# jianzhnie/ScaleRL

Measured on AMD Instinct MI355X. Metric: env_steps_per_sec, higher is better.
Workload: dtype bf16; 1 GPU; model=IMPALA AtariNet (3conv+FC512+2xLSTM519), algo=impala-vtrace, rollout_length=80, global_batch=256, seq_len=80, envs_per_actor=256, actors_per_rank=24, inference=gpu, parallelism=dp1

## Files before the change

### scalerl_amd/models/atari.py

```python

from __future__ import annotations

from typing import Dict, Tuple

import torch
import torch.nn as nn
import torch.nn.functional as F

from ..ops import MaskedLSTM, frame_cast


class AtariNet(nn.Module):
    def __init__(self, observation_shape=(4, 84, 84), num_actions: int = 6,
                 use_lstm: bool = True, native_conv: bool = None):
        super().__init__()
        self.observation_shape = tuple(observation_shape)
        self.num_actions = num_actions
        self.use_lstm = use_lstm
        if native_conv is None:
            import os
            native_conv = bool(os.environ.get("SCALERL_NATIVE_CONV"))
        self.native_conv = native_conv and tuple(observation_shape) == (4, 84, 84)

        c = observation_shape[0]
        self.conv1 = nn.Conv2d(c, 32, kernel_size=8, stride=4)
        self.conv2 = nn.Conv2d(32, 64, kernel_size=4, stride=2)
        self.conv3 = nn.Conv2d(64, 64, kernel_size=3, stride=1)
        conv_out = 64 * 7 * 7
        self.fc = nn.Linear(conv_out, 512)

        core_output_size = 512 + num_actions + 1
        if use_lstm:
            self.core = MaskedLSTM(core_output_size, core_output_size,
                                   num_layers=2)
        self.policy = nn.Linear(core_output_size, num_actions)
        self.baseline = nn.Linear(core_output_size, 1)

    def initial_state(self, batch_size: int, device=None):
        if not self.use_lstm:
            return tuple()
        return self.core.initial_state(batch_size, device=device)

    def encode(self, x: torch.Tensor) -> torch.Tensor:
        if self.native_conv and x.is_cuda:
            from ..ops.conv import native_conv
            h = native_conv(1, x, self.conv1.weight, self.conv1.bias)
            h = native_conv(2, h, self.conv2.weight, self.conv2.bias)
            h = native_conv(3, h, self.conv3.weight, self.conv3.bias)
            return F.relu(self.fc(torch.flatten(h, 1)))
        if (x.is_cuda and x.dtype == torch.uint8 and
                frame_cast.bf16_autocast_active()):
            x = frame_cast.frame_to_bf16(x)
        else:
            x = x.float() / 255.0
        x = F.relu(self.conv1(x))
        x = F.relu(self.conv2(x))
        x = F.relu(self.conv3(x))
        x = torch.flatten(x, 1)
        return F.relu(self.fc(x))

    def forward(self, inputs: Dict[str, torch.Tensor],
                core_state: Tuple = (), greedy: bool = False):
        obs = inputs["obs"]
        T, B = obs.shape[:2]
        feat = self.encode(obs.flatten(0, 1))

        one_hot_action = F.one_hot(
            inputs["last_action"].view(T * B), self.num_actions).float()
        clipped_reward = torch.clamp(inputs["reward"].view(T * B, 1), -1, 1)
        core_input = torch.cat(
            [feat.float(), clipped_reward, one_hot_action], dim=-1)

        if self.use_lstm:
            notdone = (~inputs["done"].view(T, B)).float()
            core_output, core_state = self.core(
                core_input.view(T, B, -1), notdone, core_state)
            core_output = core_output.flatten(0, 1)
        else:
            core_output = core_input

        if core_output.is_cuda:
            with torch.autocast(device_type="cuda", enabled=False):
                policy_logits = self.policy(core_output.float())
                baseline = self.baseline(core_output.float())
        else:
            policy_logits = self.policy(core_output.float())
            baseline = self.baseline(core_output.float())
        if greedy or not self.training:
            action = torch.argmax(policy_logits, dim=-1)
        else:
            action = torch.multinomial(
                F.softmax(policy_logits, dim=-1), num_samples=1).squeeze(-1)
        return ({"policy_logits": policy_logits.view(T, B, self.num_actions),
                 "baseline": baseline.view(T, B),
                 "action": action.view(T, B)}, core_state)


class AtariQNet(nn.Module):

    def __init__(self, observation_shape=(4, 84, 84), num_actions: int = 6,
                 dueling: bool = True, noisy: bool = False):
        super().__init__()
        from .noisy import NoisyLinear
        c = observation_shape[0]
        self.num_actions = num_actions
        self.dueling = dueling
        self.noisy = noisy
        lin = NoisyLinear if noisy else nn.Linear
        self.conv1 = nn.Conv2d(c, 32, kernel_size=8, stride=4)
        self.conv2 = nn.Conv2d(32, 64, kernel_size=4, stride=2)
        self.conv3 = nn.Conv2d(64, 64, kernel_size=3, stride=1)
        self.fc = nn.Linear(64 * 7 * 7, 512)
        if dueling:
            self.value_head = lin(512, 1)
            self.adv_head = lin(512, num_actions)
        else:
            self.head = lin(512, num_actions)

    def reset_noise(self):
        from .noisy import reset_noise
        reset_noise(self)

    def forward(self, x: torch.Tensor) -> torch.Tensor:
        x = x.float() / 255.0
        x = F.relu(self.conv1(x))
        x = F.relu(self.conv2(x))
        x = F.relu(self.conv3(x))
        h = F.relu(self.fc(torch.flatten(x, 1)))
        if self.dueling:
            v = self.value_head(h)
            a = self.adv_head(h)
            return v + a - a.mean(dim=-1, keepdim=True)
        return self.head(h)


class CategoricalAtariQNet(nn.Module):

    def __init__(self, observation_shape=(4, 84, 84), num_actions: int = 6,
                 num_atoms: int = 51, v_min: float = -10.0,
                 v_max: float = 10.0, noisy: bool = False):
        super().__init__()
        from .noisy import NoisyLinear
        c = observation_shape[0]
        self.action_dim = self.num_actions = num_actions
        self.num_atoms = num_atoms
        self.noisy = noisy
        lin = NoisyLinear if noisy else nn.Linear
        self.conv1 = nn.Conv2d(c, 32, kernel_size=8, stride=4)
        self.conv2 = nn.Conv2d(32, 64, kernel_size=4, stride=2)
        self.conv3 = nn.Conv2d(64, 64, kernel_size=3, stride=1)
        self.fc = nn.Linear(64 * 7 * 7, 512)
        self.head = lin(512, num_actions * num_atoms)
        self.register_buffer("support", torch.linspace(v_min, v_max, num_atoms))
        self.v_min, self.v_max = v_min, v_max
        self.delta_z = (v_max - v_min) / (num_atoms - 1)

    def reset_noise(self):
        from .noisy import reset_noise
        reset_noise(self)

    def dist(self, x: torch.Tensor) -> torch.Tensor:
        x = x.float() / 255.0
        x = F.relu(self.conv1(x))
        x = F.relu(self.conv2(x))
        x = F.relu(self.conv3(x))
        h = F.relu(self.fc(torch.flatten(x, 1)))
        logits = self.head(h).view(-1, self.num_actions, self.num_atoms)
        return F.log_softmax(logits, dim=-1)

    def forward(self, x: torch.Tensor) -> torch.Tensor:
        return (self.dist(x).exp() * self.support).sum(-1)
```

### scalerl_amd/ops/__init__.py

```python

from ._backend import available as kernels_available
from ._backend import build as build_kernels
from .frame_cast import frame_to_bf16
from .lstm import MaskedLSTM
from .optim import FusedAdam, FusedRMSprop, clip_grad_norm_, fused_polyak_
from .per import SumTree
from .scans import discounted_returns, gae, nstep_fold
from .td import fused_td_loss, per_is_weights, td_loss_reference
from .ppo import ppo_fused_loss, ppo_loss_reference
from .vtrace import (VTraceReturns, action_log_probs, impala_loss,
                     impala_loss_reference, vtrace_from_log_rhos,
                     vtrace_reference)

__all__ = [
    "kernels_available", "build_kernels", "MaskedLSTM", "FusedAdam",
    "FusedRMSprop", "clip_grad_norm_", "fused_polyak_", "SumTree",
    "discounted_returns", "gae", "nstep_fold", "fused_td_loss",
    "per_is_weights", "td_loss_reference", "VTraceReturns",
    "action_log_probs", "impala_loss", "impala_loss_reference",
    "vtrace_from_log_rhos", "vtrace_reference", "ppo_fused_loss",
    "ppo_loss_reference", "frame_to_bf16",
]
```

### scalerl_amd/ops/csrc/frame_cast.hip

```cpp

#include "common.h"

#include <stdint.h>

__device__ __forceinline__ uint32_t frame_bf16_bits(uint32_t byte) {
  const float f = (float)byte * (1.0f / 255.0f);
  uint32_t u = __float_as_uint(f);
  u += 0x7fffu + ((u >> 16) & 1u);
  return u >> 16;
}

__device__ __forceinline__ uint32_t frame_bf16_pair(uint32_t word, int k) {
  const uint32_t lo = frame_bf16_bits((word >> (16 * k)) & 0xffu);
  const uint32_t hi = frame_bf16_bits((word >> (16 * k + 8)) & 0xffu);
  return lo | (hi << 16);
}

extern "C" __global__ void frame_cast_u8_bf16_kernel(
    const uint8_t* __restrict__ in,
    uint16_t* __restrict__ out,
    long n_vec,
    long n) {
  const long tid = (long)blockIdx.x * blockDim.x + threadIdx.x;
  const long stride = (long)gridDim.x * blockDim.x;
  const uint4* in4 = reinterpret_cast<const uint4*>(in);
  uint4* out4 = reinterpret_cast<uint4*>(out);
  for (long v = tid; v < n_vec; v += stride) {
    const uint4 p = in4[v];
    uint4 a, b;
    a.x = frame_bf16_pair(p.x, 0);
    a.y = frame_bf16_pair(p.x, 1);
    a.z = frame_bf16_pair(p.y, 0);
    a.w = frame_bf16_pair(p.y, 1);
    b.x = frame_bf16_pair(p.z, 0);
    b.y = frame_bf16_pair(p.z, 1);
    b.z = frame_bf16_pair(p.w, 0);
    b.w = frame_bf16_pair(p.w, 1);
    out4[2 * v] = a;
    out4[2 * v + 1] = b;
  }
  for (long i = n_vec * 16 + tid; i < n; i += stride)
    out[i] = (uint16_t)frame_bf16_bits(in[i]);
}

extern "C" int frame_cast_u8_bf16(const void* in, void* out, long n,
                                  hipStream_t stream) {
  if (n <= 0) return 0;
  const bool aligned =
      (((uintptr_t)in | (uintptr_t)out) & (uintptr_t)15) == 0;
  const long n_vec = aligned ? n / 16 : 0;
  const int block = 256;
  const long work = n_vec > 0 ? n_vec : n;
  hipLaunchKernelGGL(frame_cast_u8_bf16_kernel, dim3(grid_1d(work, block)),
                     dim3(block), 0, stream, (const uint8_t*)in,
                     (uint16_t*)out, n_vec, n);
  CHECK_LAUNCH();
  return 0;
}
```

Baseline: 419,100 env-steps/s.

## Fuse uint8 cast and three conv layers into one persistent MFMA encoder kernel

Adds a persistent HIP kernel that converts uint8 frames to bf16 in LDS and runs conv1, conv2 and conv3 with bias and ReLU using MFMA, keeping intermediate activations in shared memory. It also prefetches the next frame while computing. It is enabled by default on the inference (no-grad) path for actor forward passes, replacing the separate cast kernel and three conv launches with their global-memory round trips. Training stays on the old path unless an env flag is set, in which case a custom backward uses the saved activations. Weights are cast to bf16 on every call, which adds small per-call overhead.

New measurement: 494,600 env-steps/s (median of 6 runs). +18.0%, better.

```diff
diff --git a/scalerl_amd/models/atari.py b/scalerl_amd/models/atari.py
--- a/scalerl_amd/models/atari.py
+++ b/scalerl_amd/models/atari.py
@@ -1,6 +1,7 @@
 
 from __future__ import annotations
 
+import os
 from typing import Dict, Tuple
 
 import torch
@@ -8,17 +9,25 @@
 import torch.nn.functional as F
 
 from ..ops import MaskedLSTM, frame_cast
+from ..ops.encoder import fused_encoder
+
+FUSED_ENCODER = os.environ.get("SCALERL_FUSED_ENCODER", "1") != "0"
+FUSED_ENCODER_TRAIN = os.environ.get("SCALERL_FUSED_ENCODER_TRAIN", "0") == "1"
 
 
 class AtariNet(nn.Module):
     def __init__(self, observation_shape=(4, 84, 84), num_actions: int = 6,
-                 use_lstm: bool = True, native_conv: bool = None):
+                 use_lstm: bool = True, native_conv: bool = None,
+                 fused_encoder: bool = None):
         super().__init__()
         self.observation_shape = tuple(observation_shape)
         self.num_actions = num_actions
         self.use_lstm = use_lstm
+        if fused_encoder is None:
+            fused_encoder = native_conv is not False
+        self.fused_encoder = (bool(fused_encoder) and
+                              tuple(observation_shape) == (4, 84, 84))
         if native_conv is None:
-            import os
             native_conv = bool(os.environ.get("SCALERL_NATIVE_CONV"))
         self.native_conv = native_conv and tuple(observation_shape) == (4, 84, 84)
 
@@ -48,8 +57,16 @@
             h = native_conv(2, h, self.conv2.weight, self.conv2.bias)
             h = native_conv(3, h, self.conv3.weight, self.conv3.bias)
             return F.relu(self.fc(torch.flatten(h, 1)))
-        if (x.is_cuda and x.dtype == torch.uint8 and
-                frame_cast.bf16_autocast_active()):
+        bf16_frames = (x.is_cuda and x.dtype == torch.uint8 and
+                       frame_cast.bf16_autocast_active())
+        if (bf16_frames and self.fused_encoder and FUSED_ENCODER and
+                (FUSED_ENCODER_TRAIN or not torch.is_grad_enabled()) and
+                x.is_contiguous() and x.data_ptr() % 16 == 0):
+            h = fused_encoder(x, self.conv1.weight, self.conv1.bias,
+                              self.conv2.weight, self.conv2.bias,
+                              self.conv3.weight, self.conv3.bias)
+            return F.relu(self.fc(torch.flatten(h, 1)))
+        if bf16_frames:
             x = frame_cast.frame_to_bf16(x)
         else:
             x = x.float() / 255.0
diff --git a/scalerl_amd/ops/__init__.py b/scalerl_amd/ops/__init__.py
--- a/scalerl_amd/ops/__init__.py
+++ b/scalerl_amd/ops/__init__.py
@@ -1,6 +1,7 @@
 
 from ._backend import available as kernels_available
 from ._backend import build as build_kernels
+from .encoder import fused_encoder
 from .frame_cast import frame_to_bf16
 from .lstm import MaskedLSTM
 from .optim import FusedAdam, FusedRMSprop, clip_grad_norm_, fused_polyak_
@@ -19,5 +20,5 @@
     "per_is_weights", "td_loss_reference", "VTraceReturns",
     "action_log_probs", "impala_loss", "impala_loss_reference",
     "vtrace_from_log_rhos", "vtrace_reference", "ppo_fused_loss",
-    "ppo_loss_reference", "frame_to_bf16",
+    "ppo_loss_reference", "frame_to_bf16", "fused_encoder",
 ]
diff --git a/scalerl_amd/ops/csrc/encoder_fwd.hip b/scalerl_amd/ops/csrc/encoder_fwd.hip
--- /dev/null
+++ b/scalerl_amd/ops/csrc/encoder_fwd.hip
@@ -0,0 +1,302 @@
+
+#include "common.h"
+#include "frame_cast.h"
+
+typedef __bf16 bf16_t;
+typedef float f32x4 __attribute__((ext_vector_type(4)));
+typedef bf16_t bf16x8 __attribute__((ext_vector_type(8)));
+typedef bf16_t bf16x4 __attribute__((ext_vector_type(4)));
+typedef uint32_t u32x4 __attribute__((ext_vector_type(4)));
+
+namespace {
+
+constexpr int ENC_IMG_BYTES = 4 * 84 * 84;
+constexpr int ENC_CH_EL = 48 * 84;
+constexpr int ENC_IMG_EL = 4 * ENC_CH_EL;
+constexpr int ENC_ACT1_EL = 32 * 400;
+constexpr int ENC_P3 = 72;
+constexpr int ENC_ACT2_EL = 81 * ENC_P3;
+constexpr int ENC_OUT3_EL = 64 * 49;
+static_assert(ENC_ACT2_EL <= ENC_IMG_EL, "act2 aliases the image range");
+static_assert((ENC_IMG_EL + ENC_ACT1_EL + ENC_OUT3_EL) * 2 <= 65536,
+              "static LDS cap");
+
+template <int H>
+struct Half {
+  static constexpr int R0 = H ? 40 : 0;
+  static constexpr int NROWS = H ? 44 : 48;
+  static constexpr int VEC = NROWS * 84 / 16;
+  static constexpr int TILE0 = H ? 13 : 0;
+  static constexpr int NTILES = H ? 12 : 13;
+  static_assert(NROWS * 84 % 16 == 0 && R0 * 84 % 16 == 0, "16-byte chunks");
+  static_assert(VEC <= 256, "one load per thread and channel");
+};
+
+template <int H>
+__device__ __forceinline__ void load_half(const uint8_t* __restrict__ ximg,
+                                          uint4 (&pre)[4], int tid) {
+  if (tid < Half<H>::VEC) {
+    #pragma unroll
+    for (int c = 0; c < 4; ++c)
+      pre[c] = reinterpret_cast<const uint4*>(
+          ximg + c * (84 * 84) + Half<H>::R0 * 84)[tid];
+  }
+}
+
+template <int H>
+__device__ __forceinline__ void store_half(const uint4 (&pre)[4],
+                                           bf16_t* img, int tid) {
+  if (tid < Half<H>::VEC) {
+    #pragma unroll
+    for (int c = 0; c < 4; ++c) {
+      uint4 a, b;
+      frame_bf16_x16(pre[c], a, b);
+      uint4* dst = reinterpret_cast<uint4*>(img + c * ENC_CH_EL);
+      dst[2 * tid] = a;
+      dst[2 * tid + 1] = b;
+    }
+  }
+}
+
+__device__ __forceinline__ bf16x4 relu_bias_pack(const f32x4 acc, float bias) {
+  bf16x4 o;
+  #pragma unroll
+  for (int r = 0; r < 4; ++r) o[r] = (bf16_t)fmaxf(acc[r] + bias, 0.f);
+  return o;
+}
+
+template <int H>
+__device__ __forceinline__ void conv1_half(const bf16_t* img, bf16_t* act1,
+                                           const bf16x8 (&B1)[8], float bias,
+                                           int wave, int g, int lr) {
+  const int nt = wave >> 1;
+  for (int t = wave & 1; t < Half<H>::NTILES; t += 4) {
+    const bool two = t + 2 < Half<H>::NTILES;
+    const int tile[2] = {Half<H>::TILE0 + t,
+                         Half<H>::TILE0 + (two ? t + 2 : t)};
+    int base[2];
+    #pragma unroll
+    for (int i = 0; i < 2; ++i) {
+      const int px = tile[i] * 16 + lr;
+      const int oy = px / 20, ox = px - oy * 20;
+      base[i] = (oy * 4 - Half<H>::R0 + g) * 84 + ox * 4;
+    }
+    f32x4 acc[2] = {{0.f, 0.f, 0.f, 0.f}, {0.f, 0.f, 0.f, 0.f}};
+    #pragma unroll
+    for (int kt = 0; kt < 8; ++kt) {
+      const int off = (kt >> 1) * ENC_CH_EL + (kt & 1) * 4 * 84;
+      #pragma unroll
+      for (int i = 0; i < 2; ++i) {
+        const bf16x4* p = reinterpret_cast<const bf16x4*>(img + base[i] + off);
+        const bf16x8 a =
+            __builtin_shufflevector(p[0], p[1], 0, 1, 2, 3, 4, 5, 6, 7);
+        acc[i] = __builtin_amdgcn_mfma_f32_16x16x32_bf16(a, B1[kt], acc[i],
+                                                         0, 0, 0);
+      }
+    }
+    bf16_t* row = act1 + (nt * 16 + lr) * 400 + g * 4;
+    *reinterpret_cast<bf16x4*>(row + tile[0] * 16) =
+        relu_bias_pack(acc[0], bias);
+    if (two)
+      *reinterpret_cast<bf16x4*>(row + tile[1] * 16) =
+          relu_bias_pack(acc[1], bias);
+  }
+}
+
+template <bool SAVE>
+__global__ __launch_bounds__(256) __attribute__((amdgpu_waves_per_eu(2)))
+void atari_encoder_fwd_kernel(
+    const uint8_t* __restrict__ x,
+    const bf16_t* __restrict__ w1,
+    const float* __restrict__ b1,
+    const bf16_t* __restrict__ w2,
+    const float* __restrict__ b2,
+    const bf16_t* __restrict__ w3,
+    const float* __restrict__ b3,
+    bf16_t* __restrict__ out1,
+    bf16_t* __restrict__ out2,
+    bf16_t* __restrict__ out3,
+    long batch) {
+  __shared__ __attribute__((aligned(16)))
+  bf16_t lds[ENC_IMG_EL + ENC_ACT1_EL + ENC_OUT3_EL];
+  bf16_t* const img = lds;
+  bf16_t* const act2 = lds;
+  bf16_t* const act1 = lds + ENC_IMG_EL;
+  bf16_t* const o3 = lds + ENC_IMG_EL + ENC_ACT1_EL;
+
+  const int tid = threadIdx.x;
+  const int wave = tid >> 6;
+  const int lane = tid & (WAVE - 1);
+  const int g = lane >> 4, lr = lane & 15;
+
+  const int ch1 = (wave >> 1) * 16 + lr;
+  const int ch = wave * 16 + lr;
+  bf16x8 B1[8], B2[16], B3[18];
+  #pragma unroll
+  for (int kt = 0; kt < 8; ++kt)
+    B1[kt] = *reinterpret_cast<const bf16x8*>(w1 + ch1 * 256 + kt * 32 + g * 8);
+  #pragma unroll
+  for (int kt = 0; kt < 16; ++kt)
+    B2[kt] = *reinterpret_cast<const bf16x8*>(w2 + ch * 512 + kt * 32 + g * 8);
+  #pragma unroll
+  for (int kt = 0; kt < 18; ++kt) {
+    #pragma unroll
+    for (int j = 0; j < 8; ++j)
+      B3[kt][j] = w3[ch * 576 + ((kt & 1) * 32 + g * 8 + j) * 9 + (kt >> 1)];
+  }
+  const float bias1 = b1[ch1], bias2 = b2[ch], bias3 = b3[ch];
+
+  int base2[6], base3[4];
+  #pragma unroll
+  for (int mt = 0; mt < 6; ++mt) {
+    const int px = min(mt * 16 + lr, 80);
+    const int oy = px / 9, ox = px - oy * 9;
+    base2[mt] = (g >> 1) * 400 + (oy * 2 + (g & 1) * 2) * 20 + ox * 2;
+  }
+  #pragma unroll
+  for (int mt = 0; mt < 4; ++mt) {
+    const int px = min(mt * 16 + lr, 48);
+    const int oy = px / 7, ox = px - oy * 7;
+    base3[mt] = (oy * 9 + ox) * ENC_P3 + g * 8;
+  }
+
+  long n = blockIdx.x;
+  uint4 pre[4];
+  if (n < batch) load_half<0>(x + n * ENC_IMG_BYTES, pre, tid);
+
+  for (; n < batch; n += gridDim.x) {
+    const uint8_t* ximg = x + n * ENC_IMG_BYTES;
+
+    store_half<0>(pre, img, tid);
+    load_half<1>(ximg, pre, tid);
+    __syncthreads();
+    conv1_half<0>(img, act1, B1, bias1, wave, g, lr);
+    __syncthreads();
+    store_half<1>(pre, img, tid);
+    __syncthreads();
+    conv1_half<1>(img, act1, B1, bias1, wave, g, lr);
+    __syncthreads();
+
+    if (SAVE) {
+      uint4* dst = reinterpret_cast<uint4*>(out1 + n * ENC_ACT1_EL);
+      const uint4* src = reinterpret_cast<const uint4*>(act1);
+      for (int i = tid; i < ENC_ACT1_EL / 8; i += 256) dst[i] = src[i];
+    }
+
+    {
+      f32x4 acc[6];
+      #pragma unroll
+      for (int mt = 0; mt < 6; ++mt) acc[mt] = (f32x4){0.f, 0.f, 0.f, 0.f};
+      #pragma unroll
+      for (int kt = 0; kt < 16; ++kt) {
+        #pragma unroll
+        for (int mt = 0; mt < 6; ++mt) {
+          const uint32_t* q = reinterpret_cast<const uint32_t*>(
+              act1 + base2[mt] + kt * 800);
+          const u32x4 v = {q[0], q[1], q[10], q[11]};
+          acc[mt] = __builtin_amdgcn_mfma_f32_16x16x32_bf16(
+              __builtin_bit_cast(bf16x8, v), B2[kt], acc[mt], 0, 0, 0);
+        }
+      }
+      #pragma unroll
+      for (int mt = 0; mt < 6; ++mt) {
+        #pragma unroll
+        for (int r = 0; r < 4; ++r) {
+          const int px = mt * 16 + g * 4 + r;
+          if (px < 81)
+            act2[px * ENC_P3 + ch] = (bf16_t)fmaxf(acc[mt][r] + bias2, 0.f);
+        }
+      }
+    }
+    __syncthreads();
+
+    if (SAVE) {
+      uint4* dst = reinterpret_cast<uint4*>(out2 + n * (64 * 81));
+      const uint16_t* src = reinterpret_cast<const uint16_t*>(act2);
+      for (int v = tid; v < 64 * 81 / 8; v += 256) {
+        int c = (v * 8) / 81, px = v * 8 - c * 81;
+        uint32_t w[4];
+        #pragma unroll
+        for (int j = 0; j < 8; ++j) {
+          const uint32_t e = src[px * ENC_P3 + c];
+          w[j >> 1] = (j & 1) ? (w[j >> 1] | (e << 16)) : e;
+          if (++px == 81) { px = 0; ++c; }
+        }
+        dst[v] = make_uint4(w[0], w[1], w[2], w[3]);
+      }
+    }
+
+    if (n + gridDim.x < batch)
+      load_half<0>(x + (n + gridDim.x) * ENC_IMG_BYTES, pre, tid);
+
+    {
+      f32x4 acc[4];
+      #pragma unroll
+      for (int mt = 0; mt < 4; ++mt) acc[mt] = (f32x4){0.f, 0.f, 0.f, 0.f};
+      #pragma unroll
+      for (int kt = 0; kt < 18; ++kt) {
+        const int tap = kt >> 1;
+        const int off = ((tap / 3) * 9 + tap % 3) * ENC_P3 + (kt & 1) * 32;
+        #pragma unroll
+        for (int mt = 0; mt < 4; ++mt) {
+          const bf16x8 a =
+              *reinterpret_cast<const bf16x8*>(act2 + base3[mt] + off);
+          acc[mt] = __builtin_amdgcn_mfma_f32_16x16x32_bf16(a, B3[kt], acc[mt],
+                                                            0, 0, 0);
+        }
+      }
+      #pragma unroll
+      for (int mt = 0; mt < 4; ++mt) {
+        #pragma unroll
+        for (int r = 0; r < 4; ++r) {
+          const int px = mt * 16 + g * 4 + r;
+          if (px < 49)
+            o3[ch * 49 + px] = (bf16_t)fmaxf(acc[mt][r] + bias3, 0.f);
+        }
+      }
+    }
+    __syncthreads();
+
+    {
+      uint4* dst = reinterpret_cast<uint4*>(out3 + n * ENC_OUT3_EL);
+      const uint4* src = reinterpret_cast<const uint4*>(o3);
+      for (int i = tid; i < ENC_OUT3_EL / 8; i += 256) dst[i] = src[i];
+    }
+  }
+}
+
+}
+
+extern "C" int atari_encoder_fwd(const void* x, const void* w1,
+                                 const float* b1, const void* w2,
+                                 const float* b2, const void* w3,
+                                 const float* b3, void* out1, void* out2,
+                                 void* out3, long batch, hipStream_t stream) {
+  if (batch <= 0) return 0;
+  if ((out1 == nullptr) != (out2 == nullptr)) return (int)hipErrorInvalidValue;
+  static int n_cu = 0;
+  if (n_cu == 0) {
+    int dev = 0, v = 0;
+    if (hipGetDevice(&dev) != hipSuccess ||
+        hipDeviceGetAttribute(&v, hipDeviceAttributeMultiprocessorCount,
+                              dev) != hipSuccess || v <= 0)
+      v = 256;
+    n_cu = v;
+  }
+  const long resident = 2L * n_cu;
+  const unsigned grid = (unsigned)(batch < resident ? batch : resident);
+  if (out1) {
+    hipLaunchKernelGGL(atari_encoder_fwd_kernel<true>, dim3(grid), dim3(256),
+                       0, stream, (const uint8_t*)x, (const bf16_t*)w1, b1,
+                       (const bf16_t*)w2, b2, (const bf16_t*)w3, b3,
+                       (bf16_t*)out1, (bf16_t*)out2, (bf16_t*)out3, batch);
+  } else {
+    hipLaunchKernelGGL(atari_encoder_fwd_kernel<false>, dim3(grid), dim3(256),
+                       0, stream, (const uint8_t*)x, (const bf16_t*)w1, b1,
+                       (const bf16_t*)w2, b2, (const bf16_t*)w3, b3,
+                       (bf16_t*)nullptr, (bf16_t*)nullptr, (bf16_t*)out3,
+                       batch);
+  }
+  CHECK_LAUNCH();
+  return 0;
+}
diff --git a/scalerl_amd/ops/csrc/frame_cast.h b/scalerl_amd/ops/csrc/frame_cast.h
--- /dev/null
+++ b/scalerl_amd/ops/csrc/frame_cast.h
@@ -0,0 +1,29 @@
+#pragma once
+
+#include <hip/hip_runtime.h>
+#include <stdint.h>
+
+__device__ __forceinline__ uint32_t frame_bf16_bits(uint32_t byte) {
+  const float f = (float)byte * (1.0f / 255.0f);
+  uint32_t u = __float_as_uint(f);
+  u += 0x7fffu + ((u >> 16) & 1u);
+  return u >> 16;
+}
+
+__device__ __forceinline__ uint32_t frame_bf16_pair(uint32_t word, int k) {
+  const uint32_t lo = frame_bf16_bits((word >> (16 * k)) & 0xffu);
+  const uint32_t hi = frame_bf16_bits((word >> (16 * k + 8)) & 0xffu);
+  return lo | (hi << 16);
+}
+
+__device__ __forceinline__ void frame_bf16_x16(const uint4 p, uint4& a,
+                                               uint4& b) {
+  a.x = frame_bf16_pair(p.x, 0);
+  a.y = frame_bf16_pair(p.x, 1);
+  a.z = frame_bf16_pair(p.y, 0);
+  a.w = frame_bf16_pair(p.y, 1);
+  b.x = frame_bf16_pair(p.z, 0);
+  b.y = frame_bf16_pair(p.z, 1);
+  b.z = frame_bf16_pair(p.w, 0);
+  b.w = frame_bf16_pair(p.w, 1);
+}
diff --git a/scalerl_amd/ops/csrc/frame_cast.hip b/scalerl_amd/ops/csrc/frame_cast.hip
--- a/scalerl_amd/ops/csrc/frame_cast.hip
+++ b/scalerl_amd/ops/csrc/frame_cast.hip
@@ -1,20 +1,6 @@
 
 #include "common.h"
-
-#include <stdint.h>
-
-__device__ __forceinline__ uint32_t frame_bf16_bits(uint32_t byte) {
-  const float f = (float)byte * (1.0f / 255.0f);
-  uint32_t u = __float_as_uint(f);
-  u += 0x7fffu + ((u >> 16) & 1u);
-  return u >> 16;
-}
-
-__device__ __forceinline__ uint32_t frame_bf16_pair(uint32_t word, int k) {
-  const uint32_t lo = frame_bf16_bits((word >> (16 * k)) & 0xffu);
-  const uint32_t hi = frame_bf16_bits((word >> (16 * k + 8)) & 0xffu);
-  return lo | (hi << 16);
-}
+#include "frame_cast.h"
 
 extern "C" __global__ void frame_cast_u8_bf16_kernel(
     const uint8_t* __restrict__ in,
@@ -28,14 +14,7 @@
   for (long v = tid; v < n_vec; v += stride) {
     const uint4 p = in4[v];
     uint4 a, b;
-    a.x = frame_bf16_pair(p.x, 0);
-    a.y = frame_bf16_pair(p.x, 1);
-    a.z = frame_bf16_pair(p.y, 0);
-    a.w = frame_bf16_pair(p.y, 1);
-    b.x = frame_bf16_pair(p.z, 0);
-    b.y = frame_bf16_pair(p.z, 1);
-    b.z = frame_bf16_pair(p.w, 0);
-    b.w = frame_bf16_pair(p.w, 1);
+    frame_bf16_x16(p, a, b);
     out4[2 * v] = a;
     out4[2 * v + 1] = b;
   }
diff --git a/scalerl_amd/ops/encoder.py b/scalerl_amd/ops/encoder.py
--- /dev/null
+++ b/scalerl_amd/ops/encoder.py
@@ -0,0 +1,93 @@
+
+from __future__ import annotations
+
+import ctypes
+
+import torch
+
+from . import _backend, frame_cast
+
+_c = ctypes.c_void_p
+
+_W_SHAPES = ((32, 4, 8, 8), (64, 32, 4, 4), (64, 64, 3, 3))
+
+
+def _declare_encoder(lib):
+    if getattr(lib, "_encoder_declared", False):
+        return lib
+    c = ctypes
+    lib.atari_encoder_fwd.argtypes = [c.c_void_p] * 10 + [c.c_long, c.c_void_p]
+    lib.atari_encoder_fwd.restype = c.c_int
+    lib._encoder_declared = True
+    return lib
+
+
+@torch.no_grad()
+def atari_encoder_fwd(x, w1, b1, w2, b2, w3, b3, save: bool):
+    assert x.is_cuda and x.dtype == torch.uint8
+    assert tuple(x.shape[1:]) == (4, 84, 84), x.shape
+    lib = _declare_encoder(_backend.lib())
+    n = x.shape[0]
+    xc = x.contiguous()
+    assert xc.data_ptr() % 16 == 0, "atari_encoder_fwd needs 16-byte aligned frames"
+    ws = [w.to(torch.bfloat16).contiguous() for w in (w1, w2, w3)]
+    bs = [b.float().contiguous() for b in (b1, b2, b3)]
+    for w, shape in zip(ws, _W_SHAPES):
+        assert w.numel() == shape[0] * shape[1] * shape[2] * shape[3], w.shape
+    dev = x.device
+    out1 = out2 = None
+    if save:
+        out1 = torch.empty((n, 32, 20, 20), dtype=torch.bfloat16, device=dev)
+        out2 = torch.empty((n, 64, 9, 9), dtype=torch.bfloat16, device=dev)
+    out3 = torch.empty((n, 64, 7, 7), dtype=torch.bfloat16, device=dev)
+    ret = lib.atari_encoder_fwd(
+        _c(xc.data_ptr()),
+        _c(ws[0].data_ptr()), _c(bs[0].data_ptr()),
+        _c(ws[1].data_ptr()), _c(bs[1].data_ptr()),
+        _c(ws[2].data_ptr()), _c(bs[2].data_ptr()),
+        _c(out1.data_ptr()) if save else None,
+        _c(out2.data_ptr()) if save else None,
+        _c(out3.data_ptr()), n, _backend.current_stream())
+    _backend.check(ret, "atari_encoder_fwd")
+    del xc, ws, bs
+    return out1, out2, out3
+
+
+class _FusedEncoderFn(torch.autograd.Function):
+
+    @staticmethod
+    def forward(ctx, x, w1, b1, w2, b2, w3, b3):
+        save = any(ctx.needs_input_grad)
+        wb = [w.detach().to(torch.bfloat16).contiguous() for w in (w1, w2, w3)]
+        out1, out2, out3 = atari_encoder_fwd(
+            x, wb[0], b1.detach(), wb[1], b2.detach(), wb[2], b3.detach(),
+            save)
+        if save:
+            ctx.save_for_backward(x, wb[0], wb[1], wb[2], out1, out2, out3)
+        return out3
+
+    @staticmethod
+    @torch.autograd.function.once_differentiable
+    def backward(ctx, dout):
+        x, wb1, wb2, wb3, out1, out2, out3 = ctx.saved_tensors
+        conv_bwd = torch.ops.aten.convolution_backward
+
+        def layer_bwd(g, inp, w, stride, mask):
+            return conv_bwd(g, inp, w, [w.shape[0]], [stride, stride], [0, 0],
+                            [1, 1], False, [0, 0], 1, mask)
+
+        relu_bwd = torch.ops.aten.threshold_backward
+
+        g3 = relu_bwd(dout.to(torch.bfloat16), out3, 0)
+        d2, dw3, db3 = layer_bwd(g3, out2, wb3, 1, [True, True, True])
+        g2 = relu_bwd(d2, out2, 0)
+        d1, dw2, db2 = layer_bwd(g2, out1, wb2, 2, [True, True, True])
+        g1 = relu_bwd(d1, out1, 0)
+        xb = frame_cast.frame_to_bf16(x)
+        _, dw1, db1 = layer_bwd(g1, xb, wb1, 4, [False, True, True])
+        return (None, dw1.float(), db1.float(), dw2.float(), db2.float(),
+                dw3.float(), db3.float())
+
+
+def fused_encoder(x, w1, b1, w2, b2, w3, b3) -> torch.Tensor:
+    return _FusedEncoderFn.apply(x, w1, b1, w2, b2, w3, b3)
```
